# baoe/AlignGraph

Measured on AMD Instinct MI355X. Metric: aligned reads/sec through graph build+extend, higher is better.
Workload: dtype u32

## Files before the change

### aligngraph_amd/csrc/agx_walk.cpp

```cpp
#include "agx_host.h"

#include <algorithm>
#include <atomic>
#include <thread>
#include <chrono>
#include <cstdio>
#include <cstdlib>
#include <cstring>
#include <deque>
#include <memory>
#include <memory_resource>
#include <string>
#include <vector>
#include <unordered_map>
#if defined(__x86_64__)
#include <immintrin.h>
#endif

#if defined(AGX_WALK_PROF) && defined(__x86_64__)
#include <x86intrin.h>
static unsigned long long g_prof[12];
#define AGX_PT(i) do { _mm_lfence(); const unsigned long long t_ = __rdtsc(); g_prof[i] += t_ - tp_; tp_ = t_; } while (0)
#define AGX_PT_START _mm_lfence(); unsigned long long tp_ = __rdtsc()
#else
// ... 16 lines not shown
};
struct Rec {
    int extended;
    agx_u32 sID, sOff, eID, eOff, sID0, sOff0, eID0, eOff0;
    Bases nuc;
    explicit Rec(Arena *a) : nuc(a) {}
};

inline char *put_u32(char *w, agx_u32 v) {
    char t[10]; int n = 0;
    do { t[n++] = (char)('0' + v % 10u); v /= 10u; } while (v);
    while (n) *w++ = t[--n];
    return w;
}

struct LineWriter {
    char *w; unsigned col = 0;
    explicit LineWriter(char *at) : w(at) {}
    void put(const char *p, size_t n) {
        if (col) {
            const size_t m = n < 60u - col ? n : 60u - col;
            memcpy(w, p, m); w += m; p += m; n -= m; col += (unsigned)m;
            if (col < 60u) return;
            *w++ = '\n'; col = 0;
        }
        for (; n >= 64; n -= 60, p += 60, w += 61) { memcpy(w, p, 64); w[60] = '\n'; }
        if (n >= 60) { memcpy(w, p, 60); w[60] = '\n'; w += 61; p += 60; n -= 60; }
        memcpy(w, p, n); w += n; col = (unsigned)n;
    }
    void put(const Bases &b) { for (const Seg &g : b.segs) put(g.p, g.n); }
    char *end() { if (col) { *w++ = '\n'; col = 0; } return w; }
};

struct PreJob { agx_u32 f[10]; const Seg *segs; size_t n_segs, total; };
inline void format_pre(OutBuf &out, const PreJob &j) {
    char hdr[256];
    char *h = hdr; *h++ = '>';
    for (int i = 0; i < 10; i++) { h = put_u32(h, j.f[i]); if (i < 9) { *h++ = ','; *h++ = ' '; } }
    *h++ = ' '; *h++ = '\n';
    const size_t hl = (size_t)(h - hdr), lines = (j.total + 59) / 60;
    char *w = out.grow(hl + j.total + lines); memcpy(w, hdr, hl);
    LineWriter lw(w + hl); for (size_t i = 0; i < j.n_segs; i++) lw.put(j.segs[i].p, j.segs[i].n); lw.end();
}
inline void note_paths(const PreJob &j, const GraphView &G, WalkPaths &P) {
    size_t off = 0; bool prev = false;
    for (size_t i = 0; i < j.n_segs; i++) {
        const Seg &g = j.segs[i];
        const bool in = g.n && g.p >= G.str && g.p < G.str + G.n_ids;
        if (in) {
            const agx_u32 a = (agx_u32)(g.p - G.str);
            P.id_first.push_back(a); P.id_last.push_back(a + (agx_u32)g.n - 1u); P.base_off.push_back(off); P.joined.push_back(prev ? 1 : 0);
        }
        prev = in; off += g.n;
    }
    P.rec_len.push_back(j.total); P.st_end.push_back(P.id_first.size());
}
struct PreFormat {
    OutBuf &out; Assistant *assistant;
    std::vector<PreJob> jobs, late; size_t cap = 0;
    std::atomic<size_t> published{0}; std::atomic<bool> finished{false}, failed{false};
    WalkPaths *paths = nullptr; const GraphView *graph = nullptr;
    PreFormat(OutBuf &o, Assistant *a, size_t capacity) : out(o), assistant(a), cap(a ? capacity : 0) {
        if (!assistant) return;
        jobs.reserve(cap);
        assistant->run([this] {
            try {
                size_t at = 0; unsigned idle = 0;
                for (;;) {
                    const size_t n = published.load(std::memory_order_acquire);
                    if (at < n) { while (at < n) format_pre(out, jobs[at++]); idle = 0; continue; }
                    if (finished.load(std::memory_order_acquire) && at == published.load(std::memory_order_acquire)) return;
                    if (++idle < 64) {
#if defined(__x86_64__)
                        _mm_pause();
#endif
                    } else std::this_thread::sleep_for(std::chrono::microseconds(20));
                }
            } catch (...) { failed.store(true); }
        });
    }
    void add(const PreJob &j) {
        if (paths) note_paths(j, *graph, *paths);
        if (!assistant) { format_pre(out, j); return; }
        if (jobs.size() < cap) { jobs.push_back(j); published.store(jobs.size(), std::memory_order_release); }
        else late.push_back(j);
    }
    void finish() {
        if (!assistant) return;
        finished.store(true, std::memory_order_release);
        assistant->wait();
        if (failed.load()) throw Error{E_ARG, "out of host memory"};
        for (const PreJob &j : late) format_pre(out, j);
        late.clear();
    }
    ~PreFormat() { if (assistant && !finished.load()) { finished.store(true, std::memory_order_release); assistant->wait(); } }
};

inline bool contains(agx_u32 sID1, agx_u32 sOff1, agx_u32 eID1, agx_u32 eOff1, agx_u32 sID2, agx_u32 sOff2, agx_u32 eID2, agx_u32 eOff2) {
    return sID1 == sID2 && eID1 == eID2 && sOff1 <= sOff2 && eOff1 >= eOff2;
}


#define AGX_WM_VISITED AGX_WM_ABSENT
inline agx_u32 run_end_scalar(const agx_u8 *meta, agx_u32 j, agx_u8 &seen) {
    for (;;) {
        uint64_t mw, dw; memcpy(&mw, meta + j, 8); memcpy(&dw, meta + j + 1, 8);
        if ((mw & 0x0101010101010101ull) == 0x0101010101010101ull && (dw & 0x8080808080808080ull) == 0) { mw |= mw >> 32; mw |= mw >> 16; mw |= mw >> 8; seen |= (agx_u8)mw; j += 8; continue; }
        for (int b8 = 0; b8 < 8; b8++) { const agx_u8 m = meta[j]; seen |= m; if (!(m & AGX_WM_CONT) || (meta[j + 1] & AGX_WM_VISITED)) return j; j++; }
    }
}
inline void mark_scalar(agx_u8 *meta, agx_u32 a, agx_u32 b) { for (agx_u32 i = a; i <= b; i++) meta[i] |= AGX_WM_VISITED; }
#if defined(__x86_64__)
__attribute__((target("avx2"))) inline agx_u32 run_end_avx2(const agx_u8 *meta, agx_u32 j, agx_u8 &seen) {
    unsigned contig = 0;
    for (;;) {
        const __m256i m = _mm256_loadu_si256((const __m256i *)(meta + j)), d = _mm256_loadu_si256((const __m256i *)(meta + j + 1));
        const unsigned pass = (unsigned)_mm256_movemask_epi8(_mm256_slli_epi16(m, 7)) & ~(unsigned)_mm256_movemask_epi8(d);
        const unsigned stop = ~pass;
        const unsigned cbits = (unsigned)_mm256_movemask_epi8(_mm256_slli_epi16(m, 6));
        if (stop == 0) { contig |= cbits; j += 32; continue; }
        const unsigned k = (unsigned)__builtin_ctz(stop);
        contig |= cbits & (k == 31 ? 0xFFFFFFFFu : ((2u << k) - 1u));
        if (contig) seen |= AGX_WM_CONTIG;
        return j + k;
    }
}
__attribute__((target("avx2"))) inline void mark_avx2(agx_u8 *meta, agx_u32 a, agx_u32 b) {
    const agx_u32 n = b - a + 1;
// ... 174 lines not shown
            for (agx_u32 i = 0; i < len; i++) {
                const agx_u32 j = rev ? first - i : first + i;
                char c = "ACGT"[(row[j >> 2] >> (2u * (j & 3u))) & 3u];
                if (c == 'A' && V.n_other) {
                    const unsigned long long *e = V.other_idx + V.n_other, *at = std::lower_bound(V.other_idx, e, base + j);
                    if (at != e && *at == base + j) c = (char)V.other_byte[at - V.other_idx];
                }
                out.push_back(!rev ? c : c == 'A' ? 'T' : c == 'C' ? 'G' : c == 'G' ? 'C' : c == 'T' ? 'A' : c);
            }
            return;
        }
        const char *p = V.row_off ? V.bases + V.row_off[r.slot] : V.bases + (size_t)(G.row_slot ? G.row_slot[r.slot] : r.slot) * V.stride;
        for (agx_u32 i = 0; i < len; i++) {
            if (!rev) out.push_back(p[first + i]);
            else { const char c = p[first - i]; out.push_back(c == 'A' ? 'T' : c == 'C' ? 'G' : c == 'G' ? 'C' : c == 'T' ? 'A' : c); }
        }
    }
    next_zero_fn next_zero = pick_next_zero();
    agx_u32 next_live(agx_u32 from, agx_u32 n) const { return from < n ? next_zero(m, from, n) : n; }
};

struct WalkState {
    agx_u32 cp = 0;
    agx_u32 seqID = 0, sIDBak = AGX_NONE, sOffBak = AGX_NONE, eIDBak = AGX_NONE, eOffBak = AGX_NONE;
    agx_u32 pos_bak = 0;
    bool same_scan(const WalkState &o) const { return cp == o.cp && sIDBak == o.sIDBak && sOffBak == o.sOffBak && eIDBak == o.eIDBak && eOffBak == o.eOffBak && pos_bak == o.pos_bak; }
};
typedef std::vector<std::pair<agx_u32, agx_u32>> MarkLog;

struct WalkRun {
    Walker &W; Arena *arena;
    WalkState st;
    std::vector<Rec> &written; PreFormat *pre;
    std::vector<PreJob> jobs;
    bool keep = true;
    MarkLog *log = nullptr; agx_u32 log_main = 0, log_side = 0;
    const std::atomic<bool> *cancel = nullptr;
    unsigned long long n_walks = 0, n_hops = 0, n_runs = 0, n_general = 0, run_nodes = 0;
    WalkRun(Walker &w, Arena *a, std::vector<Rec> &out, PreFormat *p) : W(w), arena(a), written(out), pre(p) {}
    void note_marks(agx_u32 a, agx_u32 b) {
        if (a < W.G.n_pos) { if (b >= log_main) log->push_back({a < log_main ? log_main : a, b}); }
        else if (b >= log_side) log->push_back({a < log_side ? log_side : a, b});
    }
    void go(agx_u32 stop) {
        const GraphView &G = W.G; const UnitView &V = W.V;
        agx_u32 &seqID = st.seqID, &sIDBak = st.sIDBak, &sOffBak = st.sOffBak, &eIDBak = st.eIDBak, &eOffBak = st.eOffBak, &pos_bak = st.pos_bak;
        std::string kmer; agx_u32 klen = 0, klast = 0;
        agx_hop hcur{0, 0, 0};
        std::vector<Seg> segs;
        agx_u8 *const m = W.m;
        auto done = [m, this](agx_u32 v) { AGX_WCHK(W, v, "done"); (void)this; return (m[v] & AGX_WM_VISITED) != 0; };
        const mark_fn mark = pick_mark();
        AGX_PT_START;
        const run_end_fn run_end = pick_run_end();
        const agx_u32 n_side = G.n_ids - G.n_pos;
        if (stop > G.n_pos) stop = G.n_pos;
        agx_u32 sc = (agx_u32)(std::lower_bound(G.side_xpos, G.side_xpos + n_side, st.cp) - G.side_xpos);
        agx_u32 side_live = G.n_pos + sc, main_live = st.cp;
        agx_u32 cp = st.cp;
        for (; cp < stop;) {
            if (W.invalid || (cancel && cancel->load(std::memory_order_relaxed))) break;
            while (sc < n_side && G.side_xpos[sc] < cp) sc++;
            agx_u32 sh = sc; while (sh < n_side && G.side_xpos[sh] == cp) sh++;
            const agx_u32 s_lo = G.n_pos + sc, s_hi = G.n_pos + sh;
            for (agx_u32 vi = 0, start = cp; vi <= s_hi - s_lo; vi++, start = s_lo + vi - 1) {
                if (done(start)) continue;
                AGX_PT(8);
// ... 32 lines not shown
                        mark(m, cur, j);
                        if (log && j >= log_main) note_marks(cur, j);
                        if (j > cur) pos_bak = xj;
                        cur = j; last = j; cpp = xj;
                        AGX_PT(3);
                        agx_u32 tgt = 0;
                        const int ns = (m[cur] & AGX_WM_CONT) ? 0 : W.live_successors(cur, tgt);
                        if (ns == 1) { cur = tgt; pos_bak = W.pos_of(tgt); cpp = pos_bak; }
                        else if ((hcur = W.hop_of(j, xj)).len) mode = 0;
                        else mode = -1;
                        AGX_PT(4);
                    }
                }
                C.eID = 0; C.eOff = mode == 1 ? pos_bak : cpp;
                if (mode == 1 || mode == -1) {
                    { const agx_u32 o = W.node(cur).off0; C.eID0 = o == AGX_NONE ? AGX_NONE : 0; C.eOff0 = o; }
                    klen = (W.node(last).sref.qlen >> 16) & 0x7FFFu; klast = last;
                    C.eOff = C.eOff + klen - 1; C.eOff0 = C.eOff0 + klen - 1;
                } else { C.eID0 = AGX_NONE; C.eOff0 = AGX_NONE; klen = 0; }
                AGX_PT(5);
                if (!contains(sIDBak, sOffBak, eIDBak, eOffBak, C.sID, C.sOff, C.eID, C.eOff)) {
                    { const agx_u32 o = W.node(start).off0; C.sID0 = o == AGX_NONE ? AGX_NONE : 0; C.sOff0 = o; }
                    if (klen > 1) {
                        W.kmer_string(klast, kmer);
                        char *t = (char *)arena->allocate(kmer.size() - 1, 1); memcpy(t, kmer.data() + 1, kmer.size() - 1);
                        segs.push_back(Seg{t, kmer.size() - 1});
                    }
                    C.nuc.segs.reserve(segs.size());
                    for (const Seg &g : segs) C.nuc.add(g.p, g.n);
                    sIDBak = C.sID; sOffBak = C.sOff; eIDBak = C.eID; eOffBak = C.eOff;
                    if (eOffBak - sOffBak > 100000) W.prefetch_skip_positions(cp, eOffBak < G.n_pos ? eOffBak : G.n_pos);
                    if (keep) {
                        PreJob j; const agx_u32 f[10] = {seqID, (agx_u32)C.extended, C.sID, C.sOff, C.eID, C.eOff, C.sID0, C.sOff0, C.eID0, C.eOff0};
                        memcpy(j.f, f, sizeof f); j.segs = C.nuc.segs.data(); j.n_segs = C.nuc.segs.size(); j.total = C.nuc.len;
                        if (pre) pre->add(j); else jobs.push_back(j);
                        written.push_back(std::move(C));
                    }
                    seqID++;
                }
                AGX_PT(6);
            }
            AGX_PT(9);
            if (eOffBak - sOffBak > 100000 && eIDBak == 0 && cp + 1000 < eOffBak) cp += 1000;
            else {
                auto stale = [m](agx_u32 v) { return (m[v] & AGX_WM_VISITED) != 0; };
                if (main_live <= cp || (main_live < G.n_pos && stale(main_live))) main_live = W.next_live(main_live > cp + 1 ? main_live : cp + 1, G.n_pos);
                const agx_u32 m = main_live;
                if (side_live < s_hi || (side_live < G.n_ids && stale(side_live))) side_live = W.next_live(side_live > s_hi ? side_live : s_hi, G.n_ids);
                const agx_u32 sd = side_live;
                const agx_u32 sp = sd < G.n_ids ? G.side_xpos[sd - G.n_pos] : G.n_pos;
                cp = m < sp ? m : sp;
                if (cp >= W.scan_hi) { W.invalid = true; W.gave_up_at = cp; }
            }
            AGX_PT(10);
    }
        st.cp = cp;
    }
};

inline void walk_report(const WalkRun &r) {
#if defined(AGX_WALK_PROF) && defined(__x86_64__)
    if (getenv("AGX_WALK_TIMING")) {
        fprintf(stderr, "[agx walk] Mcycles: start %.1f, hop %.1f, run scan %.1f, mark %.1f, successors %.1f, end %.1f, contain+write %.1f, between %.1f, position scan %.1f (+ %.1f after the last variant, %.1f next position)\n",
                g_prof[0] / 1e6, g_prof[1] / 1e6, g_prof[2] / 1e6, g_prof[3] / 1e6, g_prof[4] / 1e6, g_prof[5] / 1e6, g_prof[6] / 1e6, g_prof[7] / 1e6, g_prof[8] / 1e6, g_prof[9] / 1e6, g_prof[10] / 1e6);
        memset(g_prof, 0, sizeof g_prof);
    }
#endif
    if (getenv("AGX_WALK_TIMING")) fprintf(stderr, "[agx walk] walks %llu, contig hops %llu, runs %llu (%llu nodes), general evaluations %llu\n", r.n_walks, r.n_hops, r.n_runs, r.run_nodes, r.n_general);
}

void walk(Walker &W, OutBuf &pre_out, std::vector<Rec> &written, Arena *arena, Assistant *assistant, WalkPaths *paths) {
    if (W.G.wait_landed) W.G.wait_landed(W.G.land_ctx, W.G.n_pos, W.G.n_ids);
    if (W.G.wait_str) W.G.wait_str(W.G.land_ctx);
    pre_out.reserve((size_t)W.G.n_ids + W.G.n_ids / 32 + 4096);
    PreFormat pre(pre_out, assistant, (size_t)W.G.n_pos / 256 + 65536);
    pre.paths = paths; pre.graph = &W.G;
    WalkRun run(W, arena, written, &pre);
    run.go(W.G.n_pos);
    pre.finish();
    walk_report(run);
}

inline std::atomic<double> &walker_speed() { static std::atomic<double> v{700000.0}; return v; }
inline void clip_marks(const MarkLog &log, agx_u32 main_lo, agx_u32 main_hi, agx_u32 n_pos, agx_u32 side_lo, agx_u32 side_hi, MarkLog &out) {
    out.clear();
    for (const auto &r : log) {
        agx_u32 a = r.first, b = r.second;
        if (b < n_pos) { if (a < main_lo) a = main_lo; if (b >= main_hi) { if (main_hi == 0) continue; b = main_hi - 1; } }
        else { if (a < side_lo) a = side_lo; if (b >= side_hi) { if (side_hi == 0) continue; b = side_hi - 1; } }
        if (a <= b) out.push_back({a, b});
    }
    std::sort(out.begin(), out.end());
    size_t k = 0;
    for (size_t i = 0; i < out.size(); i++) {
        if (k && out[i].first <= out[k - 1].second + 1) { if (out[i].second > out[k - 1].second) out[k - 1].second = out[i].second; }
        else out[k++] = out[i];
    }
    out.resize(k);
}

struct SpecWalker {
    agx_u32 c = 0, c_next = 0, w0 = 0, side_c = 0, side_next = 0, warm_lo = 0, warm_hi = 0xFFFFFFFFu, look_hi = 0, win_lo = 0, win_hi = 0, side_win_hi = 0, copy_hi = 0, side_copy_lo = 0, side_copy_hi = 0;
    Scratch bytes;
    GraphView G; std::unique_ptr<Walker> W; std::unique_ptr<WalkRun> R; std::vector<Rec> recs;
    MarkLog log; size_t n_warm = 0;
    WalkState at_c;
    bool ok = false; std::string error;
    double t_run = 0, t_copy = 0, t_warm = 0, t_done = 0;
};

bool walk_split(Walker &WA, const UnitView &V, const GraphView &G, OutBuf &pre_out, std::vector<Rec> &written, Arena *arena, Arena *const *more_arenas, Assistant *assistant, WalkPaths *paths) {
    const agx_u32 min_ref = getenv("AGX_WALK_SPLIT_MIN") ? (agx_u32)strtoul(getenv("AGX_WALK_SPLIT_MIN"), nullptr, 10) : 4000000u;
    agx_u32 warm = 400000u;
    if (const char *e = getenv("AGX_WALK_SPLIT_WARMUP")) warm = (agx_u32)strtoul(e, nullptr, 10);
    else if (V.segs) {
        agx_u32 reach = 0;
        for (agx_u32 i = 0; i < V.n_seg0; i++) { const agx_cmseg &g = V.segs[i]; if (g.hop_len0 && g.hop_end > g.pos0 && g.hop_end - g.pos0 > reach) reach = g.hop_end - g.pos0; }
        const unsigned long long w = 3ull * reach + 20000ull;
        warm = (agx_u32)(w < 100000ull ? 100000ull : w > 400000ull ? 400000ull : w);
    }
    const agx_u32 n_ref = V.n_ref < G.n_pos ? V.n_ref : G.n_pos;
    if (!assistant || n_ref < min_ref || n_ref < 16 || getenv("AGX_WALK_NO_SPLIT")) return false;
    int K = walkers_for(n_ref);
    if (K > 1 + assistant->helpers()) K = 1 + assistant->helpers();
    const agx_u32 slack = 64;
    if (K > (int)(n_ref / (8 * slack))) K = (int)(n_ref / (8 * slack));
    if (K < 2) return false;
    const agx_u32 lead = n_ref / (unsigned)K > 4 * warm ? 2 * warm : 0;
    std::vector<agx_u32> cuts((size_t)K + 1, n_ref); cuts[0] = 0;
    for (int i = 1; i < K; i++) cuts[(size_t)i] = lead + (agx_u32)((unsigned long long)(n_ref - lead) * (unsigned)i / (unsigned)K);
    const bool streamed = G.wait_landed != nullptr && G.land_ms > 0;
    if (!getenv("AGX_WALK_EVEN_CUTS")) {
        const double v = walker_speed().load(), D = streamed ? G.land_ms : 0.0, copy_ms = 0.15 + 3.2 * ((double)n_ref / K) / 12e6, warm_ms = 2.0 * (double)warm / v, floor_len = std::max(1024.0, (double)n_ref / (16.0 * K));
        std::vector<double> len((size_t)K, (double)n_ref / K), ready((size_t)K, 0.0), at((size_t)K + 1, 0.0);
        for (int round = 0; round < 6; round++) {
            for (int i = 0; i < K; i++) at[(size_t)i + 1] = at[(size_t)i] + len[(size_t)i];
            double sum = ready[0] = D;
            for (int i = 1; i < K; i++) { const double hi = i + 2 >= K ? (double)G.n_pos : std::max(at[(size_t)i + 2], at[(size_t)i + 1] + (double)warm); sum += ready[(size_t)i] = D * std::min(1.0, hi / (double)G.n_pos) + copy_ms + warm_ms; }
            const double T = ((double)n_ref / v + sum) / K;
            double total = 0;
            for (int i = 0; i < K; i++) total += len[(size_t)i] = std::max(v * (T - ready[(size_t)i]), floor_len);
            for (int i = 0; i < K; i++) len[(size_t)i] *= (double)n_ref / total;
        }
        double acc = 0;
        for (int i = 1; i < K; i++) { acc += len[(size_t)i - 1]; const agx_u32 lo = cuts[(size_t)i - 1] + 8 * slack, hi = n_ref - (agx_u32)(K - i) * 8 * slack; const agx_u32 c = (agx_u32)acc; cuts[(size_t)i] = c < lo ? lo : c > hi ? hi : c; }
    }
    auto cut_at = [&](int i) { return i >= K ? n_ref : i <= 0 ? 0u : cuts[(size_t)i]; };
    const agx_u32 n_side = G.n_ids - G.n_pos;
    auto side_of = [&](agx_u32 x) { return G.n_pos + (agx_u32)(std::lower_bound(G.side_xpos, G.side_xpos + n_side, x) - G.side_xpos); };
    const agx_u32 side_ref = side_of(n_ref);
    pre_out.reserve((size_t)G.n_ids + G.n_ids / 32 + 4096);
    const bool timing = getenv("AGX_WALK_TIMING") != nullptr;
    auto clock = [] { return std::chrono::duration<double, std::milli>(std::chrono::steady_clock::now().time_since_epoch()).count(); };

    const double t_enter = clock();
    std::atomic<bool> cancel{false};
    std::atomic<int> copied{0};
    const agx_u8 *const pristine = WA.m;
    std::vector<SpecWalker> B((size_t)K - 1);
    for (int i = 1; i < K; i++) {
        SpecWalker &b = B[(size_t)i - 1];
        b.c = cut_at(i); b.c_next = cut_at(i + 1);
        b.side_c = side_of(b.c); b.side_next = side_of(b.c_next);
        int ahead = i + 2; while (ahead < K && cut_at(ahead) < b.c_next + warm) ahead++;
        const bool open_end = ahead >= K;
        const agx_u32 back = 2 * warm + slack < b.c - cut_at(i - 1) ? 2 * warm + slack : b.c - cut_at(i - 1);
        b.win_lo = b.c - back; b.win_hi = open_end ? n_ref : cut_at(ahead); b.side_win_hi = open_end ? side_ref : side_of(b.win_hi);
        b.copy_hi = open_end ? G.n_pos : b.win_hi; b.side_copy_lo = side_of(b.win_lo); b.side_copy_hi = open_end ? G.n_ids : b.side_win_hi;
        b.warm_lo = b.win_lo ? b.win_lo + slack : 0; b.warm_hi = open_end ? 0xFFFFFFFFu : b.win_hi - slack; b.look_hi = open_end ? n_ref : b.win_hi - slack;
        b.w0 = b.c > warm ? b.c - warm : 0; if (b.w0 < b.warm_lo) b.w0 = b.warm_lo;
        b.bytes.take((size_t)G.n_ids + 64);
        b.G = G; b.G.meta = (const agx_u8 *)b.bytes.p; b.G.meta_rw = (agx_u8 *)b.bytes.p;
        b.W.reset(new Walker(V, b.G));
        b.recs.reserve((size_t)G.n_pos / 2048 + 1024);
        b.R.reset(new WalkRun(*b.W, more_arenas[i - 1], b.recs, nullptr));
    }
    struct Join { Assistant *a; int n; std::atomic<bool> &c; std::vector<bool> joined; void now(int i) { if (!joined[(size_t)i]) { a->wait(i); joined[(size_t)i] = true; } } ~Join() { c.store(true); for (int i = 0; i < n; i++) now(i); } } join{assistant, K - 1, cancel, std::vector<bool>((size_t)K - 1, false)};
    for (int i = 1; i < K; i++) {
        SpecWalker *bp = &B[(size_t)i - 1];
        assistant->run([bp, &cancel, &copied, pristine, &G, n_ref, side_ref] {
            SpecWalker &b = *bp; Walker &W = *b.W; WalkRun &R = *b.R;
            auto clk = [] { return std::chrono::duration<double, std::milli>(std::chrono::steady_clock::now().time_since_epoch()).count(); };
            b.t_run = clk();
            struct Copied { std::atomic<int> &n; bool done = false; void now() { if (!done) { done = true; n.fetch_add(1, std::memory_order_release); } } ~Copied() { now(); } } copied_mark{copied};
// ... 23 lines not shown
        }, i - 1);
    }
    WA.copies = &copied; WA.copies_want = K - 1; WA.guard_main = B[0].win_lo; WA.guard_side = B[0].side_copy_lo;
    struct Unguard { Walker &w; ~Unguard() { w.copies = nullptr; } } unguard{WA};
    if (G.wait_landed) G.wait_landed(G.land_ctx, G.n_pos, G.n_ids);

    const double tw0 = clock();
    MarkLog log_a;
    WalkRun A(WA, arena, written, nullptr);
    A.log = &log_a; A.log_main = B[0].c; A.log_side = B[0].side_c;
    A.go(B[0].c);
    A.log = nullptr;
    const size_t a_first = A.jobs.size();
    const double tw1 = clock();
    const MarkLog *truth = &log_a; WalkState at = A.st; int stood = 0; MarkLog ma, mb;
    for (int i = 1; i < K; i++) {
        SpecWalker &b = B[(size_t)i - 1];
        join.now(i - 1);
        bool same = b.ok && b.error.empty() && at.same_scan(b.at_c);
        if (same) {
            MarkLog warm_marks(b.log.begin(), b.log.begin() + (long)b.n_warm);
            clip_marks(*truth, b.c, n_ref, G.n_pos, b.side_c, side_ref, ma); clip_marks(warm_marks, b.c, n_ref, G.n_pos, b.side_c, side_ref, mb);
            same = ma == mb;
        }
        if (timing) {
            if (same) fprintf(stderr, "[agx walk] walker %d of %d, [%u, %u) after a warm-up from %u: its stretch stands (began at %.2f ms, window %.2f ms, warm-up %.2f ms, stretch %.2f ms)\n", i + 1, K, b.c, b.c_next, b.w0, b.t_run - t_enter, b.t_copy - b.t_run, b.t_warm - b.t_copy, b.t_done - b.t_warm);
            else if (!b.error.empty()) fprintf(stderr, "[agx walk] walker %d of %d failed (%s): walked on by the first walker from %u\n", i + 1, K, b.error.c_str(), b.c);
            else if (b.W->invalid) fprintf(stderr, "[agx walk] walker %d of %d gave up (a walk led to position %u, outside [%u, %u)): walked on by the first walker from %u\n", i + 1, K, b.W->gave_up_at, b.W->look_lo, b.W->look_hi, b.c);
            else fprintf(stderr, "[agx walk] walker %d of %d, [%u, %u) after a warm-up from %u: states differ at the meeting point (scan at %u / %u, last record %u..%u / %u..%u, %zu / %zu mark ranges): walked on by the first walker\n",
                         i + 1, K, b.c, b.c_next, b.w0, at.cp, b.at_c.cp, at.sOffBak, at.eOffBak, b.at_c.sOffBak, b.at_c.eOffBak, ma.size(), mb.size());
        }
        if (!same) break;
        const agx_u32 shift = at.seqID;
        for (PreJob &j : b.R->jobs) j.f[0] += shift;
        at = b.R->st; at.seqID = shift + b.R->st.seqID;
        truth = &b.log; stood = i;
    }
    cancel.store(true);
    for (int i = stood; i < K - 1; i++) join.now(i);
    WA.copies = nullptr;
    {
        double pos = 0, ms = 0;
        for (int i = 1; i <= stood; i++) { const SpecWalker &b = B[(size_t)i - 1]; if (b.t_done > b.t_warm) { pos += (double)(b.c_next - b.c); ms += b.t_done - b.t_warm; } }
        if (ms > 0.05 && pos > 1e5) { const double seen = pos / ms, old = walker_speed().load(); walker_speed().store(0.7 * old + 0.3 * std::min(std::max(seen, 1e5), 5e6)); }
    }
    const double tw2 = clock();
    if (!(stood == K - 1 && WA.next_live(n_ref, G.n_pos) >= G.n_pos && WA.next_live(side_ref, G.n_ids) >= G.n_ids)) {
        auto merge = [&WA](const agx_u8 *src, agx_u32 lo, agx_u32 hi) {
            agx_u32 v = lo;
            for (; v < hi && (v & 7u); v++) WA.m[v] |= (agx_u8)(src[v] & AGX_WM_VISITED);
            for (; v + 8 <= hi; v += 8) { uint64_t x, y; memcpy(&x, WA.m + v, 8); memcpy(&y, src + v, 8); x |= y & 0x8080808080808080ull; memcpy(WA.m + v, &x, 8); }
            for (; v < hi; v++) WA.m[v] |= (agx_u8)(src[v] & AGX_WM_VISITED);
        };
        auto merge_of = [&](int i) {
            const SpecWalker &b = B[(size_t)i - 1]; const agx_u8 *src = b.W->m;
            if (i < stood) { merge(src, b.c, b.c_next); merge(src, b.side_c, b.side_next); } else { merge(src, b.c, b.win_hi); merge(src, b.side_c, b.side_win_hi); }
        };
        struct Wait { Assistant *a; int n; ~Wait() { for (int i = 0; i < n; i++) a->wait(i); } } wait{assistant, stood > 1 ? stood - 1 : 0};
        for (int i = 1; i < stood; i++) assistant->run([&merge_of, i] { merge_of(i); }, i - 1);
        if (stood) merge_of(stood);
    }
    for (int i = 1; i <= stood; i++) {
        SpecWalker &b = B[(size_t)i - 1];
        for (Rec &r : b.recs) written.push_back(std::move(r));
        WA.n_fetched += b.W->n_fetched;
        A.n_walks += b.R->n_walks; A.n_hops += b.R->n_hops; A.n_runs += b.R->n_runs; A.n_general += b.R->n_general; A.run_nodes += b.R->run_nodes;
    }
    if (stood) A.st = at;
    const double tw3 = clock();
    A.go(G.n_pos);
    const double tw4 = clock();
    std::vector<PreJob> all;
    all.insert(all.end(), A.jobs.begin(), A.jobs.begin() + (long)a_first);
    for (int i = 1; i <= stood; i++) all.insert(all.end(), B[(size_t)i - 1].R->jobs.begin(), B[(size_t)i - 1].R->jobs.end());
    all.insert(all.end(), A.jobs.begin() + (long)a_first, A.jobs.end());
    if (paths) for (const PreJob &j : all) note_paths(j, G, *paths);
    std::vector<size_t> place(all.size() + 1, 0);
    auto header_len = [](const PreJob &j) { size_t n = 1 + 9 * 2 + 2; for (int i = 0; i < 10; i++) { agx_u32 v = j.f[i]; do { n++; v /= 10u; } while (v); } return n; };
    for (size_t i = 0; i < all.size(); i++) place[i + 1] = place[i] + header_len(all[i]) + all[i].total + (all[i].total + 59) / 60;
    const size_t total = place[all.size()];
    if (G.wait_str) G.wait_str(G.land_ctx);
    pre_out.n = 0; char *base = pre_out.grow(total);
    auto format = [&](size_t lo, size_t hi) {
        for (size_t i = lo; i < hi; i++) {
            const PreJob &j = all[i];
            char *h = base + place[i]; *h++ = '>';
            for (int f = 0; f < 10; f++) { h = put_u32(h, j.f[f]); if (f < 9) { *h++ = ','; *h++ = ' '; } }
            *h++ = ' '; *h++ = '\n';
            LineWriter lw(h); for (size_t g = 0; g < j.n_segs; g++) lw.put(j.segs[g].p, j.segs[g].n); lw.end();
        }
    };
    {
        const int shares = total > (1u << 16) ? K : 1;
        std::vector<size_t> cut((size_t)shares + 1, all.size()); cut[0] = 0;
        for (int t = 1; t < shares; t++) { size_t m = cut[(size_t)t - 1]; while (m < all.size() && place[m] < total / (unsigned)shares * (unsigned)t) m++; cut[(size_t)t] = m; }
        struct Wait { Assistant *a; int n; ~Wait() { for (int i = 0; i < n; i++) a->wait(i); } } wait{assistant, shares - 1};
        for (int t = 0; t + 1 < shares; t++) { const size_t lo = cut[(size_t)t], hi = cut[(size_t)t + 1]; assistant->run([&format, lo, hi] { format(lo, hi); }, t); }
        format(cut[(size_t)shares - 1], all.size());
    }
    if (timing) fprintf(stderr, "[agx walk] first walker began at %.2f ms; %u appended positions behind the reference%s\n", tw0 - t_enter, G.n_pos - n_ref, streamed ? " (streamed download: stretches cut by when their windows land)" : "");
    if (timing && streamed) { fprintf(stderr, "[agx walk] cuts (%.1f ms of download left at the start, %.0f positions per ms):", G.land_ms, walker_speed().load()); for (int i = 1; i < K; i++) fprintf(stderr, " %u", cuts[(size_t)i]); fprintf(stderr, "\n"); }
    if (timing) fprintf(stderr, "[agx walk] %d walkers, %d stretches stood: first stretch %.1f ms, waited %.1f ms for the others, merge %.1f ms, rest %.1f ms, formatting %.1f ms\n", K, stood, tw1 - tw0, tw2 - tw1, tw3 - tw2, tw4 - tw3, clock() - tw4);
    walk_report(A);
    return true;
}

}

namespace {

void join(std::vector<Rec> &c) {
    const int n = (int)c.size();
    for (int cp = 0; cp < n; cp++) if (c[cp].extended == 1)
        for (int q = cp + 1; q < n; q++) {
            if (contains(c[cp].sID, c[cp].sOff, c[cp].eID, c[cp].eOff, c[q].sID, c[q].sOff, c[q].eID, c[q].eOff)) c[q].extended = 2;
            else if (c[cp].eID != c[q].sID || c[cp].eOff < c[q].sOff) break;
        }
    for (int cp = n - 1; cp >= 0; cp--) if (c[cp].extended == 1)
        for (int q = cp - 1; q >= 0; q--) {
            if (contains(c[cp].sID, c[cp].sOff, c[cp].eID, c[cp].eOff, c[q].sID, c[q].sOff, c[q].eID, c[q].eOff)) c[q].extended = 2;
            else if (c[q].eID != c[cp].sID || c[q].eOff < c[cp].sOff) break;
        }
    for (int cp = 0; cp < n; cp++) {
        while (c[cp].extended == 1) {
            int cand = -1, ncand = 0;
            for (int q = cp + 1; q < n; q++) if (c[q].extended != 2) { if (c[cp].eOff >= c[q].sOff) { cand = q; ncand++; } else break; }
            if (ncand != 1) break;
            Rec &d = c[cand]; d.extended = 2;
            const size_t from = (size_t)(int)(c[cp].eOff - d.sOff + 1);
            if (from < d.nuc.len) c[cp].nuc.add_from(d.nuc, from);
            c[cp].eID = d.eID; c[cp].eOff = d.eOff; c[cp].eID0 = d.eID0; c[cp].eOff0 = d.eOff0;
        }
    }
}

inline int overlaps(agx_u32 x1, agx_u32 y1, agx_u32 x2, agx_u32 y2) {
    return (x1 <= x2 && x2 <= y1 && y1 <= y2 && (int)y1 - (int)x2 > 0) || (x2 <= x1 && x1 <= y2 && y2 <= y1 && (int)y2 - (int)x1 > 0) ||
           (x1 <= x2 && x2 <= y2 && y2 <= y1 && (int)y2 - (int)x2 > 0) || (x2 <= x1 && x1 <= y1 && y1 <= y2 && (int)y1 - (int)x1 > 0);
}

void scaffold(const UnitView &V, const GraphView &G, std::vector<Rec> &c, OutBuf &out, Arena *arena, Assistant *assistant) {
    std::vector<Bases> sc; sc.reserve(c.size());
    const agx_u32 n = (agx_u32)c.size();
    std::vector<agx_u32> s_off(n); agx_u32 longest = 0; bool ordered = true;
    for (agx_u32 i = 0; i < n; i++) {
        s_off[i] = c[i].sOff;
        if (i && s_off[i] < s_off[i - 1]) ordered = false;
        if (c[i].eOff < c[i].sOff) longest = 0xFFFFFFFFu; else if (c[i].eOff - c[i].sOff > longest) longest = c[i].eOff - c[i].sOff;
    }
    for (agx_u32 cp = 0; cp < n; cp++) {
        if (!(c[cp].sID != AGX_NONE && c[cp].extended == 1)) continue;
        sc.push_back(std::move(c[cp].nuc)); c[cp].nuc = Bases(arena); c[cp].sID = AGX_NONE;
        bool cont = true;
        while (c[cp].sID0 == c[cp].eID0 && cont) {
            cont = false;
            agx_u32 q = cp + 1;
            if (ordered && longest != 0xFFFFFFFFu && c[cp].sOff0 > longest) {
                const agx_u32 from = (agx_u32)(std::lower_bound(s_off.begin(), s_off.end(), c[cp].sOff0 - longest) - s_off.begin());
                if (from > q) q = from;
            }
            for (; q < n; q++) {
                if (ordered && c[q].sOff > c[cp].eOff0) break;
                if (!(c[cp].eID0 == c[q].sID && c[q].sID == c[q].eID && overlaps(c[cp].sOff0, c[cp].eOff0, c[q].sOff, c[q].eOff) && c[q].extended == 1)) continue;
                if (c[q].sOff > c[cp].eOff) {
                    const agx_u32 gap = c[q].sOff - c[cp].eOff - 1; agx_u32 covered = 0;
                    for (agx_u32 i = 0; i < gap; i++) { const agx_u32 x = c[cp].eOff + i + 1; if ((G.meta[x] & AGX_WM_ANY) || V.has_cm(x)) covered++; }
                    if (gap == 0 || (double)(int)covered / gap >= 0.5) sc.back().add(V.ref + c[cp].eOff + 1, gap);
                    else continue;
                }
                sc.back().add_from(c[q].nuc, 0); c[q].sID = AGX_NONE; cp = q; cont = true;
                break;
            }
        }
    }
    const double t_dec = std::chrono::duration<double, std::milli>(std::chrono::steady_clock::now().time_since_epoch()).count();
    std::vector<size_t> at(sc.size() + 1, 0);
    auto header = [](char *hdr, size_t i) { char *h = hdr; *h++ = '>'; char t[24]; int n = 0; do { t[n++] = (char)('0' + i % 10); i /= 10; } while (i); while (n) *h++ = t[--n]; *h++ = '\n'; return (size_t)(h - hdr); };
    for (size_t i = 0; i < sc.size(); i++) { char hdr[32]; at[i + 1] = at[i] + header(hdr, i) + sc[i].len + (sc[i].len + 59) / 60; }
    const size_t total = at[sc.size()];
    out.n = 0; char *base = out.grow(total);
    auto format = [&](size_t lo, size_t hi) {
        for (size_t i = lo; i < hi; i++) {
            char hdr[32]; const size_t hl = header(hdr, i);
            char *w = base + at[i]; memcpy(w, hdr, hl);
            LineWriter lw(w + hl); lw.put(sc[i]); lw.end();
        }
    };
    const int shares = assistant && total > (1u << 16) ? std::min(8, 1 + assistant->helpers()) : 1;
    if (shares > 1) {
        std::vector<size_t> cut((size_t)shares + 1, sc.size()); cut[0] = 0;
        for (int t = 1; t < shares; t++) { size_t m = cut[(size_t)t - 1]; while (m < sc.size() && at[m] < total / (unsigned)shares * (unsigned)t) m++; cut[(size_t)t] = m; }
        struct Wait { Assistant *a; int n; ~Wait() { for (int i = 0; i < n; i++) a->wait(i); } } wait{assistant, shares - 1};
        for (int t = 0; t + 1 < shares; t++) { const size_t lo = cut[(size_t)t], hi = cut[(size_t)t + 1]; assistant->run([&format, lo, hi] { format(lo, hi); }, t); }
        format(cut[(size_t)shares - 1], sc.size());
    } else format(0, sc.size());
    if (getenv("AGX_WALK_TIMING")) fprintf(stderr, "[agx walk] scaffold: output %.1f ms of it (%zu scaffolds, %zu bytes)\n", std::chrono::duration<double, std::milli>(std::chrono::steady_clock::now().time_since_epoch()).count() - t_dec, sc.size(), total);
}

}

void build_chains(Threads &T) {
    const size_t n = T.cm.size(), n_pos = T.ref.size();
    T.chain_off.assign(1, 0); T.chain_end_pos.clear(); T.chain_str.clear();
    T.chain_str.reserve(n);
    T.hop.assign(n_pos, agx_hop{0, 0, 0});
    std::vector<agx_u8> state(n, 0);
    auto index_of = [&](agx_u32 off, agx_u32 item) -> size_t {
        if (off >= n_pos || T.cm_start[off] + item >= T.cm_start[off + 1]) throw Error{E_ARG, "conti-mer link to a missing entry"};
        return (size_t)T.cm_start[off] + item;
    };
    for (size_t i = 0; i < n; i++) if (T.cm[i].next_off != AGX_NONE) state[index_of(T.cm[i].next_off, T.cm[i].next_item)] = 1;
    std::vector<agx_u32> pending;
    size_t visited = 0;
    T.segs.clear(); T.n_seg0 = 0;
    for (size_t x = 0; x < n_pos; x++) for (size_t h = T.cm_start[x]; h < T.cm_start[x + 1]; h++) {
        if (state[h]) continue;
        pending.clear();
        size_t c = h; agx_u32 pos = (agx_u32)x;
        const size_t seg_first = T.segs.size(), str_base = T.chain_str.size();
        for (agx_u32 i = 0;; i++) {
            if (state[c] == 2) throw Error{E_ARG, "conti-mer chains are not simple lists"};
            state[c] = 2; visited++;
            T.chain_str.push_back(T.cm[c].nuc);
            const ContiMer &m = T.cm[c];
            {
                const agx_u32 rank = (agx_u32)(c - T.cm_start[pos]);
                agx_cmseg *g = T.segs.size() > seg_first ? &T.segs.back() : nullptr;
                const bool joins = g && pos == g->pos0 + g->len && rank == g->rank && m.cid == g->cid && (g->len == 1 || m.coff == g->coff0 + g->len * g->dcoff);
                if (joins) { if (g->len == 1) g->dcoff = m.coff - g->coff0; g->len++; }
// ... 1 lines not shown
            }
            if (m.next_off == AGX_NONE) break;
            if (T.cm_start[pos + 1] - T.cm_start[pos] == 1) { T.hop[pos].str_off = (agx_u32)T.chain_str.size(); pending.push_back(pos); }
            c = index_of(m.next_off, m.next_item); pos = m.next_off;
        }
        if (T.chain_str.size() >= 0xFFFFFFFFull) throw Error{E_ARG, "conti-mer chains exceed 2^32 bases"};
        for (agx_u32 p : pending) { T.hop[p].len = (agx_u32)(T.chain_str.size() - T.hop[p].str_off); T.hop[p].end_pos = pos; }
        {   const agx_u32 last = (agx_u32)(T.chain_str.size() - str_base - 1);
            for (size_t g = seg_first; g < T.segs.size(); g++) { T.segs[g].hop_len0 = last - T.segs[g].hop_len0; T.segs[g].hop_end = pos; } }
        T.chain_end_pos.push_back(pos); T.chain_off.push_back(T.chain_str.size());
    }
    if (visited != n) throw Error{E_ARG, "conti-mer cycle"};
    std::stable_sort(T.segs.begin(), T.segs.end(), [](const agx_cmseg &a, const agx_cmseg &b) { return (a.rank != 0) != (b.rank != 0) ? a.rank == 0 : (a.rank == 0 && a.pos0 < b.pos0); });
    agx_u32 e = 0;
    for (agx_cmseg &g : T.segs) { g.elem0 = e; e += g.len; if (g.rank == 0) T.n_seg0++; }
    if (e != n) throw Error{E_ARG, "conti-mer runs do not cover the conti-mers"};
    T.n_cm = n; T.cm_cnt.resize(n_pos);
    for (size_t x = 0; x < n_pos; x++) { const agx_u32 c = T.cm_start[x + 1] - T.cm_start[x]; if (c > 255) throw Error{E_UNSUPPORTED, "more than 255 conti-mers at one position"}; T.cm_cnt[x] = (agx_u8)c; }
}

void walk_join_scaffold(const UnitView &V, const GraphView &G, UnitOutput &out, Assistant *assistant) {
    if (!V.hop && !G.sp_hop && !V.segs) throw Error{E_ARG, "conti-mer chains were not built"};
    const bool timing = getenv("AGX_WALK_TIMING") != nullptr;
    auto now = [] { return std::chrono::duration<double, std::milli>(std::chrono::steady_clock::now().time_since_epoch()).count(); };
    const double ts = now();
    Walker W(V, G);
    std::pmr::monotonic_buffer_resource arena((size_t)8 << 20);
    std::vector<std::unique_ptr<std::pmr::monotonic_buffer_resource>> others;
    Arena *more_arenas[GraphView::MAX_WALKERS - 1];
    for (int i = 0; i < GraphView::MAX_WALKERS - 1; i++) { others.emplace_back(new std::pmr::monotonic_buffer_resource((size_t)1 << 20)); more_arenas[i] = others.back().get(); }
    std::vector<Rec> recs; recs.reserve((size_t)G.n_pos / 1024 + 1024);
    double t0 = now();
    WalkPaths *paths = out.keep_paths ? &out.paths : nullptr;
    if (!walk_split(W, V, G, out.pre_extended, recs, &arena, more_arenas, assistant, paths)) walk(W, out.pre_extended, recs, &arena, assistant, paths);
    double t1 = now();
    join(recs);
    double t2 = now();
    scaffold(V, G, recs, out.extended, &arena, assistant);
    double t3 = now();
    out.n_fetched = W.n_fetched;
    if (timing) fprintf(stderr, "[agx walk] set-up %.2f ms, walk %.2f ms, join %.2f ms, scaffold %.1f ms, %zu records, %u special ids of %u, %llu records fetched\n", t0 - ts, t1 - t0, t2 - t1, t3 - t2, recs.size(), G.n_special, G.n_ids, W.n_fetched);
}

}
```

Measured before the change: 1.345 billion.

## Overlap pre-extended FASTA formatting with join and scaffold on helper threads

Formatting of the pre-extended records is moved out of the walk. Walk pieces are kept in place instead of being concatenated, output offsets are computed incrementally, and the formatting shares are handed to assistant threads that run while join and scaffold decision proceed. Scaffold output reclaims each helper slot before reusing it, and small outputs are split into more shares. This adds more bookkeeping and some risk in the offset and numbering arithmetic, such as renumbering via digit counts.

```diff
diff --git a/aligngraph_amd/csrc/agx_walk.cpp b/aligngraph_amd/csrc/agx_walk.cpp
--- a/aligngraph_amd/csrc/agx_walk.cpp
+++ b/aligngraph_amd/csrc/agx_walk.cpp
@@ -72,7 +72,9 @@
     char *end() { if (col) { *w++ = '\n'; col = 0; } return w; }
 };
 
-struct PreJob { agx_u32 f[10]; const Seg *segs; size_t n_segs, total; };
+struct PreJob { agx_u32 f[10]; const Seg *segs; size_t n_segs, total, at; };
+inline size_t digits_below(size_t x) { size_t n = x; for (size_t p = 10; p < x; p *= 10) n += x - p; return n; }
+inline size_t bytes_unnumbered(const PreJob &j) { size_t n = 1 + 9 * 2 + 2 + j.total + (j.total + 59) / 60; for (int i = 1; i < 10; i++) { agx_u32 v = j.f[i]; do { n++; v /= 10u; } while (v); } return n; }
 inline void format_pre(OutBuf &out, const PreJob &j) {
     char hdr[256];
     char *h = hdr; *h++ = '>';
@@ -99,8 +101,9 @@
     OutBuf &out; Assistant *assistant;
     std::vector<PreJob> jobs, late; size_t cap = 0;
     std::atomic<size_t> published{0}; std::atomic<bool> finished{false}, failed{false};
+    bool defer = false, done = false;
     WalkPaths *paths = nullptr; const GraphView *graph = nullptr;
-    PreFormat(OutBuf &o, Assistant *a, size_t capacity) : out(o), assistant(a), cap(a ? capacity : 0) {
+    PreFormat(OutBuf &o, Assistant *a, size_t capacity, bool deferred = false) : out(o), assistant(deferred ? nullptr : a), cap(a && !deferred ? capacity : 0), defer(deferred) {
         if (!assistant) return;
         jobs.reserve(cap);
         assistant->run([this] {
@@ -121,19 +124,100 @@
     }
     void add(const PreJob &j) {
         if (paths) note_paths(j, *graph, *paths);
-        if (!assistant) { format_pre(out, j); return; }
+        if (!assistant && !defer) { format_pre(out, j); return; }
         if (jobs.size() < cap) { jobs.push_back(j); published.store(jobs.size(), std::memory_order_release); }
         else late.push_back(j);
     }
     void finish() {
-        if (!assistant) return;
-        finished.store(true, std::memory_order_release);
-        assistant->wait();
-        if (failed.load()) throw Error{E_ARG, "out of host memory"};
+        if (done) return;
+        if (assistant) {
+            finished.store(true, std::memory_order_release);
+            assistant->wait();
+            if (failed.load()) throw Error{E_ARG, "out of host memory"};
+        }
         for (const PreJob &j : late) format_pre(out, j);
-        late.clear();
+        late.clear(); done = true;
     }
     ~PreFormat() { if (assistant && !finished.load()) { finished.store(true, std::memory_order_release); assistant->wait(); } }
+};
+
+inline bool late_format() { const char *e = getenv("AGX_WALK_LATE_FORMAT"); return e && *e && *e != '0'; }
+inline double clock_ms() { return std::chrono::duration<double, std::milli>(std::chrono::steady_clock::now().time_since_epoch()).count(); }
+
+struct PreTail {
+    OutBuf &out; Assistant *assistant; const GraphView &G; const bool late = late_format();
+    std::unique_ptr<PreFormat> pre;
+    struct Piece { const PreJob *jobs; size_t n, first, base, at0; };
+    std::vector<std::vector<PreJob>> kept; std::vector<Piece> pieces; size_t n_records = 0, total = 0; char *base = nullptr;
+    std::vector<size_t> cut;
+    int shares = 0; bool ready = false, handed = false; bool busy[GraphView::MAX_WALKERS] = {};
+    double t_ready = 0, t_first = 0, t_last = 0, t_begin[GraphView::MAX_WALKERS] = {}, t_end[GraphView::MAX_WALKERS] = {};
+    PreTail(OutBuf &o, Assistant *a, const GraphView &g) : out(o), assistant(a), G(g) { kept.reserve(GraphView::MAX_WALKERS + 1); }
+    void add_piece(size_t which, size_t lo, size_t hi, size_t end_at) {
+        if (lo >= hi) return;
+        const PreJob *j = kept[which].data() + lo; const size_t n = hi - lo;
+        pieces.push_back(Piece{j, n, n_records, total, j[0].at});
+        total += end_at - j[0].at + digits_below(n_records + n) - digits_below(n_records); n_records += n;
+    }
+    size_t place(const Piece &p, size_t i) const { return p.base + (p.jobs[i].at - p.at0) + digits_below(p.first + i) - digits_below(p.first); }
+    size_t first_at(size_t bytes) const {
+        for (const Piece &p : pieces) {
+            if (place(p, p.n - 1) < bytes) continue;
+            size_t lo = 0, hi = p.n - 1;
+            while (lo < hi) { const size_t mid = lo + (hi - lo) / 2; if (place(p, mid) < bytes) lo = mid + 1; else hi = mid; }
+            return p.first + lo;
+        }
+        return n_records;
+    }
+    template <class F> void each(size_t lo, size_t hi, F f) const {
+        for (const Piece &p : pieces) {
+            if (p.first + p.n <= lo) continue;
+            if (p.first >= hi) break;
+            for (size_t i = lo > p.first ? lo - p.first : 0; i < p.n && p.first + i < hi; i++) f(p.jobs[i], p.first + i, place(p, i));
+        }
+    }
+    void format(size_t lo, size_t hi) const {
+        each(lo, hi, [this](const PreJob &j, size_t number, size_t at) {
+            char *h = base + at; *h++ = '>';
+            h = put_u32(h, (agx_u32)number); *h++ = ','; *h++ = ' ';
+            for (int f = 1; f < 10; f++) { h = put_u32(h, j.f[f]); if (f < 9) { *h++ = ','; *h++ = ' '; } }
+            *h++ = ' '; *h++ = '\n';
+            LineWriter lw(h); for (size_t g = 0; g < j.n_segs; g++) lw.put(j.segs[g].p, j.segs[g].n); lw.end();
+        });
+    }
+    void hand_out(int slots) {
+        out.n = 0; base = out.grow(total);
+        shares = assistant && total > 4096 ? (int)std::min<size_t>((size_t)std::min(slots, (int)GraphView::MAX_WALKERS), total / 2048) : 0;
+        cut.assign((size_t)shares + 1, n_records); cut[0] = 0;
+        for (int t = 1; t < shares; t++) cut[(size_t)t] = std::max(cut[(size_t)t - 1], first_at(total / (unsigned)shares * (unsigned)t));
+        ready = true; t_ready = clock_ms();
+        if (!late) start();
+    }
+    void start() {
+        if (handed) return;
+        handed = true;
+        for (int t = 0; t < shares; t++) {
+            assistant->run([this, t] {
+                if (G.wait_str) G.wait_str(G.land_ctx);
+                t_begin[t] = clock_ms(); format(cut[(size_t)t], cut[(size_t)t + 1]); t_end[t] = clock_ms();
+            }, t);
+            busy[t] = true;
+        }
+    }
+    void free_slot(int t) {
+        if (pre) { if (!late) pre->finish(); return; }
+        if (busy[t]) { assistant->wait(t); busy[t] = false; }
+    }
+    void finish() {
+        if (pre) { pre->finish(); return; }
+        if (!ready) return;
+        if (!shares) { if (G.wait_str) G.wait_str(G.land_ctx); format(0, n_records); }
+        start();
+        for (int t = 0; t < shares; t++) free_slot(t);
+        for (int t = 0; t < shares; t++) { if (!t || t_begin[t] < t_first) t_first = t_begin[t]; if (t_end[t] > t_last) t_last = t_end[t]; }
+        ready = false;
+    }
+    ~PreTail() { for (int t = 0; t < GraphView::MAX_WALKERS; t++) if (busy[t]) assistant->wait(t); }
 };
 
 inline bool contains(agx_u32 sID1, agx_u32 sOff1, agx_u32 eID1, agx_u32 eOff1, agx_u32 sID2, agx_u32 sOff2, agx_u32 eID2, agx_u32 eOff2) {
@@ -374,7 +458,7 @@
     Walker &W; Arena *arena;
     WalkState st;
     std::vector<Rec> &written; PreFormat *pre;
-    std::vector<PreJob> jobs;
+    std::vector<PreJob> jobs; size_t job_bytes = 0;
     bool keep = true;
     MarkLog *log = nullptr; agx_u32 log_main = 0, log_side = 0;
     const std::atomic<bool> *cancel = nullptr;
@@ -473,8 +557,8 @@
                     if (eOffBak - sOffBak > 100000) W.prefetch_skip_positions(cp, eOffBak < G.n_pos ? eOffBak : G.n_pos);
                     if (keep) {
                         PreJob j; const agx_u32 f[10] = {seqID, (agx_u32)C.extended, C.sID, C.sOff, C.eID, C.eOff, C.sID0, C.sOff0, C.eID0, C.eOff0};
-                        memcpy(j.f, f, sizeof f); j.segs = C.nuc.segs.data(); j.n_segs = C.nuc.segs.size(); j.total = C.nuc.len;
-                        if (pre) pre->add(j); else jobs.push_back(j);
+                        memcpy(j.f, f, sizeof f); j.segs = C.nuc.segs.data(); j.n_segs = C.nuc.segs.size(); j.total = C.nuc.len; j.at = job_bytes;
+                        if (pre) pre->add(j); else { job_bytes += bytes_unnumbered(j); jobs.push_back(j); }
                         written.push_back(std::move(C));
                     }
                     seqID++;
@@ -510,15 +594,15 @@
     if (getenv("AGX_WALK_TIMING")) fprintf(stderr, "[agx walk] walks %llu, contig hops %llu, runs %llu (%llu nodes), general evaluations %llu\n", r.n_walks, r.n_hops, r.n_runs, r.run_nodes, r.n_general);
 }
 
-void walk(Walker &W, OutBuf &pre_out, std::vector<Rec> &written, Arena *arena, Assistant *assistant, WalkPaths *paths) {
+void walk(Walker &W, PreTail &tail, std::vector<Rec> &written, Arena *arena, Assistant *assistant, WalkPaths *paths) {
     if (W.G.wait_landed) W.G.wait_landed(W.G.land_ctx, W.G.n_pos, W.G.n_ids);
     if (W.G.wait_str) W.G.wait_str(W.G.land_ctx);
-    pre_out.reserve((size_t)W.G.n_ids + W.G.n_ids / 32 + 4096);
-    PreFormat pre(pre_out, assistant, (size_t)W.G.n_pos / 256 + 65536);
+    tail.out.reserve((size_t)W.G.n_ids + W.G.n_ids / 32 + 4096);
+    tail.pre.reset(new PreFormat(tail.out, assistant, (size_t)W.G.n_pos / 256 + 65536, tail.late));
+    PreFormat &pre = *tail.pre;
     pre.paths = paths; pre.graph = &W.G;
     WalkRun run(W, arena, written, &pre);
     run.go(W.G.n_pos);
-    pre.finish();
     walk_report(run);
 }
 
@@ -550,7 +634,7 @@
     double t_run = 0, t_copy = 0, t_warm = 0, t_done = 0;
 };
 
-bool walk_split(Walker &WA, const UnitView &V, const GraphView &G, OutBuf &pre_out, std::vector<Rec> &written, Arena *arena, Arena *const *more_arenas, Assistant *assistant, WalkPaths *paths) {
+bool walk_split(Walker &WA, const UnitView &V, const GraphView &G, PreTail &tail, std::vector<Rec> &written, Arena *arena, Arena *const *more_arenas, Assistant *assistant, WalkPaths *paths) {
     const agx_u32 min_ref = getenv("AGX_WALK_SPLIT_MIN") ? (agx_u32)strtoul(getenv("AGX_WALK_SPLIT_MIN"), nullptr, 10) : 4000000u;
     agx_u32 warm = 400000u;
     if (const char *e = getenv("AGX_WALK_SPLIT_WARMUP")) warm = (agx_u32)strtoul(e, nullptr, 10);
@@ -590,7 +674,7 @@
     const agx_u32 n_side = G.n_ids - G.n_pos;
     auto side_of = [&](agx_u32 x) { return G.n_pos + (agx_u32)(std::lower_bound(G.side_xpos, G.side_xpos + n_side, x) - G.side_xpos); };
     const agx_u32 side_ref = side_of(n_ref);
-    pre_out.reserve((size_t)G.n_ids + G.n_ids / 32 + 4096);
+    tail.out.reserve((size_t)G.n_ids + G.n_ids / 32 + 4096);
     const bool timing = getenv("AGX_WALK_TIMING") != nullptr;
     auto clock = [] { return std::chrono::duration<double, std::milli>(std::chrono::steady_clock::now().time_since_epoch()).count(); };
 
@@ -680,7 +764,6 @@
         }
         if (!same) break;
         const agx_u32 shift = at.seqID;
-        for (PreJob &j : b.R->jobs) j.f[0] += shift;
         at = b.R->st; at.seqID = shift + b.R->st.seqID;
         truth = &b.log; stood = i;
     }
@@ -718,37 +801,19 @@
     const double tw3 = clock();
     A.go(G.n_pos);
     const double tw4 = clock();
-    std::vector<PreJob> all;
-    all.insert(all.end(), A.jobs.begin(), A.jobs.begin() + (long)a_first);
-    for (int i = 1; i <= stood; i++) all.insert(all.end(), B[(size_t)i - 1].R->jobs.begin(), B[(size_t)i - 1].R->jobs.end());
-    all.insert(all.end(), A.jobs.begin() + (long)a_first, A.jobs.end());
-    if (paths) for (const PreJob &j : all) note_paths(j, G, *paths);
-    std::vector<size_t> place(all.size() + 1, 0);
-    auto header_len = [](const PreJob &j) { size_t n = 1 + 9 * 2 + 2; for (int i = 0; i < 10; i++) { agx_u32 v = j.f[i]; do { n++; v /= 10u; } while (v); } return n; };
-    for (size_t i = 0; i < all.size(); i++) place[i + 1] = place[i] + header_len(all[i]) + all[i].total + (all[i].total + 59) / 60;
-    const size_t total = place[all.size()];
-    if (G.wait_str) G.wait_str(G.land_ctx);
-    pre_out.n = 0; char *base = pre_out.grow(total);
-    auto format = [&](size_t lo, size_t hi) {
-        for (size_t i = lo; i < hi; i++) {
-            const PreJob &j = all[i];
-            char *h = base + place[i]; *h++ = '>';
-            for (int f = 0; f < 10; f++) { h = put_u32(h, j.f[f]); if (f < 9) { *h++ = ','; *h++ = ' '; } }
-            *h++ = ' '; *h++ = '\n';
-            LineWriter lw(h); for (size_t g = 0; g < j.n_segs; g++) lw.put(j.segs[g].p, j.segs[g].n); lw.end();
-        }
-    };
-    {
-        const int shares = total > (1u << 16) ? K : 1;
-        std::vector<size_t> cut((size_t)shares + 1, all.size()); cut[0] = 0;
-        for (int t = 1; t < shares; t++) { size_t m = cut[(size_t)t - 1]; while (m < all.size() && place[m] < total / (unsigned)shares * (unsigned)t) m++; cut[(size_t)t] = m; }
-        struct Wait { Assistant *a; int n; ~Wait() { for (int i = 0; i < n; i++) a->wait(i); } } wait{assistant, shares - 1};
-        for (int t = 0; t + 1 < shares; t++) { const size_t lo = cut[(size_t)t], hi = cut[(size_t)t + 1]; assistant->run([&format, lo, hi] { format(lo, hi); }, t); }
-        format(cut[(size_t)shares - 1], all.size());
-    }
+    {   const size_t a_all = A.jobs.size(), a_bytes = A.job_bytes;
+        tail.kept.push_back(std::move(A.jobs));
+        tail.add_piece(0, 0, a_first, a_first < a_all ? tail.kept[0][a_first].at : a_bytes);
+        for (int i = 1; i <= stood; i++) { WalkRun &R = *B[(size_t)i - 1].R; const size_t n = R.jobs.size(), bytes = R.job_bytes; tail.kept.push_back(std::move(R.jobs)); tail.add_piece(tail.kept.size() - 1, 0, n, bytes); }
+        tail.add_piece(0, a_first, a_all, a_bytes);
+    }
+    if (paths) tail.each(0, tail.n_records, [&](const PreJob &j, size_t, size_t) { note_paths(j, G, *paths); });
+    const double tf0 = clock();
+    tail.hand_out(K - 1);
+    if (timing) fprintf(stderr, "[agx walk] pre-extended output: records and places %.2f ms, output buffer and %d shares handed out %.2f ms (%zu records, %zu bytes)\n", tf0 - tw4, tail.shares, clock() - tf0, tail.n_records, tail.total);
     if (timing) fprintf(stderr, "[agx walk] first walker began at %.2f ms; %u appended positions behind the reference%s\n", tw0 - t_enter, G.n_pos - n_ref, streamed ? " (streamed download: stretches cut by when their windows land)" : "");
     if (timing && streamed) { fprintf(stderr, "[agx walk] cuts (%.1f ms of download left at the start, %.0f positions per ms):", G.land_ms, walker_speed().load()); for (int i = 1; i < K; i++) fprintf(stderr, " %u", cuts[(size_t)i]); fprintf(stderr, "\n"); }
-    if (timing) fprintf(stderr, "[agx walk] %d walkers, %d stretches stood: first stretch %.1f ms, waited %.1f ms for the others, merge %.1f ms, rest %.1f ms, formatting %.1f ms\n", K, stood, tw1 - tw0, tw2 - tw1, tw3 - tw2, tw4 - tw3, clock() - tw4);
+    if (timing) fprintf(stderr, "[agx walk] %d walkers, %d stretches stood: first stretch %.1f ms, waited %.1f ms for the others, merge %.1f ms, rest %.1f ms, hand-over of the output %.1f ms\n", K, stood, tw1 - tw0, tw2 - tw1, tw3 - tw2, tw4 - tw3, clock() - tw4);
     walk_report(A);
     return true;
 }
@@ -787,8 +852,8 @@
            (x1 <= x2 && x2 <= y2 && y2 <= y1 && (int)y2 - (int)x2 > 0) || (x2 <= x1 && x1 <= y1 && y1 <= y2 && (int)y1 - (int)x1 > 0);
 }
 
-void scaffold(const UnitView &V, const GraphView &G, std::vector<Rec> &c, OutBuf &out, Arena *arena, Assistant *assistant) {
-    std::vector<Bases> sc; sc.reserve(c.size());
+void scaffold_decide(const UnitView &V, const GraphView &G, std::vector<Rec> &c, std::vector<Bases> &sc, Arena *arena) {
+    sc.reserve(c.size());
     const agx_u32 n = (agx_u32)c.size();
     std::vector<agx_u32> s_off(n); agx_u32 longest = 0; bool ordered = true;
     for (agx_u32 i = 0; i < n; i++) {
@@ -821,7 +886,9 @@
             }
         }
     }
-    const double t_dec = std::chrono::duration<double, std::milli>(std::chrono::steady_clock::now().time_since_epoch()).count();
+}
+void scaffold_output(const GraphView &G, const std::vector<Bases> &sc, OutBuf &out, Assistant *assistant, PreTail &tail) {
+    const double t_dec = clock_ms();
     std::vector<size_t> at(sc.size() + 1, 0);
     auto header = [](char *hdr, size_t i) { char *h = hdr; *h++ = '>'; char t[24]; int n = 0; do { t[n++] = (char)('0' + i % 10); i /= 10; } while (i); while (n) *h++ = t[--n]; *h++ = '\n'; return (size_t)(h - hdr); };
     for (size_t i = 0; i < sc.size(); i++) { char hdr[32]; at[i + 1] = at[i] + header(hdr, i) + sc[i].len + (sc[i].len + 59) / 60; }
@@ -834,15 +901,16 @@
             LineWriter lw(w + hl); lw.put(sc[i]); lw.end();
         }
     };
-    const int shares = assistant && total > (1u << 16) ? std::min(8, 1 + assistant->helpers()) : 1;
+    const int shares = assistant && total > 4096 ? (int)std::min<size_t>((size_t)std::min(8, 1 + assistant->helpers()), total / 2048) : 1;
+    if (G.wait_str) G.wait_str(G.land_ctx);
     if (shares > 1) {
         std::vector<size_t> cut((size_t)shares + 1, sc.size()); cut[0] = 0;
         for (int t = 1; t < shares; t++) { size_t m = cut[(size_t)t - 1]; while (m < sc.size() && at[m] < total / (unsigned)shares * (unsigned)t) m++; cut[(size_t)t] = m; }
         struct Wait { Assistant *a; int n; ~Wait() { for (int i = 0; i < n; i++) a->wait(i); } } wait{assistant, shares - 1};
-        for (int t = 0; t + 1 < shares; t++) { const size_t lo = cut[(size_t)t], hi = cut[(size_t)t + 1]; assistant->run([&format, lo, hi] { format(lo, hi); }, t); }
+        for (int t = 0; t + 1 < shares; t++) { const size_t lo = cut[(size_t)t], hi = cut[(size_t)t + 1]; tail.free_slot(t); assistant->run([&format, lo, hi] { format(lo, hi); }, t); }
         format(cut[(size_t)shares - 1], sc.size());
     } else format(0, sc.size());
-    if (getenv("AGX_WALK_TIMING")) fprintf(stderr, "[agx walk] scaffold: output %.1f ms of it (%zu scaffolds, %zu bytes)\n", std::chrono::duration<double, std::milli>(std::chrono::steady_clock::now().time_since_epoch()).count() - t_dec, sc.size(), total);
+    if (getenv("AGX_WALK_TIMING")) fprintf(stderr, "[agx walk] scaffold: output %.2f ms (%zu scaffolds, %zu bytes, %d shares)\n", clock_ms() - t_dec, sc.size(), total, shares);
 }
 
 }
@@ -910,14 +978,23 @@
     std::vector<Rec> recs; recs.reserve((size_t)G.n_pos / 1024 + 1024);
     double t0 = now();
     WalkPaths *paths = out.keep_paths ? &out.paths : nullptr;
-    if (!walk_split(W, V, G, out.pre_extended, recs, &arena, more_arenas, assistant, paths)) walk(W, out.pre_extended, recs, &arena, assistant, paths);
+    std::vector<Bases> sc;
+    PreTail tail(out.pre_extended, assistant, G);
+    if (!walk_split(W, V, G, tail, recs, &arena, more_arenas, assistant, paths)) walk(W, tail, recs, &arena, assistant, paths);
     double t1 = now();
     join(recs);
     double t2 = now();
-    scaffold(V, G, recs, out.extended, &arena, assistant);
+    scaffold_decide(V, G, recs, sc, &arena);
     double t3 = now();
+    scaffold_output(G, sc, out.extended, assistant, tail);
+    double t4 = now();
+    tail.finish();
+    double t5 = now();
     out.n_fetched = W.n_fetched;
-    if (timing) fprintf(stderr, "[agx walk] set-up %.2f ms, walk %.2f ms, join %.2f ms, scaffold %.1f ms, %zu records, %u special ids of %u, %llu records fetched\n", t0 - ts, t1 - t0, t2 - t1, t3 - t2, recs.size(), G.n_special, G.n_ids, W.n_fetched);
-}
-
-}
+    if (timing) {
+        fprintf(stderr, "[agx walk] set-up %.2f ms, walk %.2f ms, join %.2f ms, scaffold decision %.2f ms, scaffold output %.2f ms, rest of the pre-extended output %.2f ms, %zu records, %u special ids of %u, %llu records fetched\n", t0 - ts, t1 - t0, t2 - t1, t3 - t2, t4 - t3, t5 - t4, recs.size(), G.n_special, G.n_ids, W.n_fetched);
+        if (tail.shares) fprintf(stderr, "[agx walk] pre-extended shares: handed out at %.2f ms of the tail, the first began %.2f ms and the last ended %.2f ms after that (join began at %.2f ms, the scaffold output at %.2f ms)\n", tail.t_ready - t0, tail.t_first - tail.t_ready, tail.t_last - tail.t_ready, t1 - t0, t3 - t0);
+    }
+}
+
+}
```

After: 1.373 billion (median of 4 runs). 1.02x the previous value.
